# KrainskiL/CGE.jl

Measured on AMD Instinct MI355X. Metric: edge_alpha_evals_per_sec, higher is better.
Workload: dtype f64

## Files before the change

### cge.jl_amd/api.py

```python
from __future__ import annotations

import atexit
import ctypes as C
import os
import sys
import weakref

import numpy as np

from .args import _SplitRule

_HERE = os.path.dirname(os.path.abspath(__file__))
_LIB_PATH = os.path.join(_HERE, "csrc", "build", "libcge_hip.so")
_lib = None

CGE_OK = 0
_CODES = {-1: "AssertionError", -2: "ErrorException: Trying to split homogenous cluster",
          -3: "ErrorException: Unexpected empty cluster generated", -4: "HIP error / no GPU",
          -5: "collective hook failed", -6: "out of memory", -7: "bad argument"}


class CGEError(RuntimeError):
    def __init__(self, code, msg=""):
        super().__init__(f"{_CODES.get(code, 'error')} (code {code}){': ' + msg if msg else ''}")
# ... 423 lines not shown
        return out

    def segment_sort_test(self, z, offsets):
        z = _f64(z)
        off = np.ascontiguousarray(offsets, dtype=np.int32)
        zs, perm = np.empty_like(z), np.empty(z.size, dtype=np.int32)
        self._check(self.L.cge_segment_sort_test(self.h, _p(z), _p(off), C.c_int64(off.size - 1), _p(zs), _p(perm)))
        return zs, perm

    def wave_tree_test(self, x):
        x = np.ascontiguousarray(x, dtype=np.float64).reshape(-1, 64)
        a, b = np.empty(x.shape[0]), np.empty(x.shape[0])
        self._check(self.L.cge_wave_tree_test(self.h, _p(x), C.c_int64(x.shape[0]), _p(a), _p(b)))
        return a, b

    def js(self, vC, vB, vI=None, internal=True):
        vC, vB = _f64(vC), _f64(vB)
        vi = None if vI is None or len(vI) == 0 else np.ascontiguousarray(vI, dtype=np.uint8)
        out = C.c_double()
        self._check(self.L.cge_js(self.h, _p(vC), _p(vB), C.c_int64(len(vC)), _p(vi), C.c_int(int(bool(internal))),
                                  C.byref(out)))
        return out.value

    def exchange_buffer(self, min_doubles):
        ptr, cap = C.c_void_p(), C.c_int64()
        self._check(self.L.cge_exchange_buffer(self.h, C.c_int64(min_doubles), C.byref(ptr), C.byref(cap)))
        return ptr.value, cap.value

    def set_collectives(self, fn, rank, world):
        cb = ALLREDUCE_FN(fn)
# ... 173 lines not shown
```

### cge.jl_amd/csrc/capi.cpp

```cpp
#include <algorithm>
#include <cmath>
#include <future>
#include <thread>
#include <unordered_set>

#include "common.hpp"
#include "../../include/cge_hip_testing.h"
#include <limits>

void k_gather_i32(cge_ctx *c, const i32 *arr, const i32 *idx, i64 S, i32 *out);

#define CGE_TRY(ctx) try {
#define CGE_CATCH(ctx)                                             \
    }                                                              \
    catch (const CgeError &e) {                                    \
        if (ctx) (ctx)->err = e.msg;                               \
        return e.code;                                             \
    }                                                              \
    catch (const std::bad_alloc &) {                               \
        if (ctx) (ctx)->err = "host allocation failed";            \
        return CGE_E_OOM;                                          \
    }                                                              \
    catch (const std::exception &e) {                              \
        if (ctx) (ctx)->err = e.what();                            \
// ... 67 lines not shown
    try {
        HIP_CHECK(hipSetDevice(device));
        c->device = device;
        if (stream) {
            c->stream = (hipStream_t)stream;
        } else {
            HIP_CHECK(hipStreamCreateWithFlags(&c->stream, hipStreamNonBlocking));
            c->own_stream = true;
        }
        HIP_CHECK(hipStreamCreateWithFlags(&c->copy_stream, hipStreamNonBlocking));
        HIP_CHECK(hipEventCreateWithFlags(&c->copy_ev, hipEventDisableTiming));
        HIP_CHECK(hipEventCreateWithFlags(&c->copy_done, hipEventDisableTiming));
        for (int i = 0; i < 2; i++) HIP_CHECK(hipEventCreateWithFlags(&c->sweep_ev[i], hipEventDisableTiming));
        for (int i = 0; i < 2; i++) HIP_CHECK(hipEventCreateWithFlags(&c->tab_ev[i], hipEventDisableTiming));
        for (int i = 0; i < 2; i++) HIP_CHECK(hipEventCreateWithFlags(&c->stage_ev[i], hipEventDisableTiming));
        unsigned hc = std::thread::hardware_concurrency();
        c->n_threads = (int)std::max(1u, std::min(hc ? hc : 8u, 16u));
        c->pool = new ThreadPool(c->n_threads - 1);
        for (int b = 0; b < 2; b++) c->stage[b].ensure(CGE_STAGE_BYTES);
        {
            DevBuf<unsigned char> warm;
            warm.ensure((size_t)1 << 20);
            for (int b = 0; b < 2; b++) {
                memset(c->stage[b].p, 0, (size_t)1 << 20);
                HIP_CHECK(hipMemcpyAsync(warm.p, c->stage[b].p, (size_t)1 << 20, hipMemcpyHostToDevice, c->stream));
            }
            HIP_CHECK(hipStreamSynchronize(c->stream));
        }
        if (const char *nap = getenv("CGE_FIT_TEST_DELAY")) {
            c->opt_fit_test_delay = std::max(0, std::min(atoi(nap), 2000));
// ... 17 lines not shown
    flush_timers(c);
    (void)cge_comm_finalize(c);
    if (c->own_stream && c->stream) (void)hipStreamDestroy(c->stream);
    if (c->copy_stream) { (void)hipStreamSynchronize(c->copy_stream); (void)hipStreamDestroy(c->copy_stream); }
    for (hipEvent_t e : c->event_pool) (void)hipEventDestroy(e);
    c->event_pool.clear();
    if (c->copy_ev) (void)hipEventDestroy(c->copy_ev);
    if (c->copy_done) (void)hipEventDestroy(c->copy_done);
    if (c->samp_ev) (void)hipEventDestroy(c->samp_ev);
    for (int i = 0; i < 2; i++) {
        if (c->sweep_ev[i]) (void)hipEventDestroy(c->sweep_ev[i]);
        if (c->tab_ev[i]) (void)hipEventDestroy(c->tab_ev[i]);
    }
    for (int i = 0; i < 2; i++)
        if (c->stage_ev[i]) (void)hipEventDestroy(c->stage_ev[i]);
    delete c->pool;
    c->pool = nullptr;
    delete c;
}

const char *cge_last_error(const cge_ctx *c) { return c ? c->err.c_str() : "null context"; }

int cge_set_host_threads(cge_ctx *c, int n) {
    if (!c || n < 1) return CGE_E_ARG;
    c->n_threads = n;
    delete c->pool;
    c->pool = new ThreadPool(n - 1);
    return CGE_OK;
}

// ... 546 lines not shown
    if (method < 0 || method > 3) CGE_THROW(CGE_E_ARG, "unknown split method %d", method);
    const i64 d = c->d;
    hipStream_t st = c->stream;
    double t0 = now_ms();
    land = clamp_to_unique_rows(c, land, &c->lm_truncated);
    c->phases.ms["lm_unique"] = now_ms() - t0;
    if (c->after_unique) {
        std::function<void()> f;
        f.swap(c->after_unique);
        f();
    }
    std::vector<i64> gid;
    host_runsplit(c, cl_flat, cl_off, ncl, land, forced, method, gid, true);
    HIP_CHECK(hipStreamSynchronize(st));
    c->phases.ms["landmarks"] = now_ms() - t0;
    t0 = now_ms();
    const i64 N = (i64)c->h_mem_off.size() - 1;
    c->N = N;
    c->h_v2l.clear();
    c->lemb.ensure((size_t)N * d);
    c->lweight.ensure(N);
    c->dii.ensure(N);
    c->lcomm.ensure(N);
    {
        ScopedKernelTimer tm(c, "landmark_aggregate");
        k_landmark_aggregate(c, c->Xr.p, lm_vw(c), lm_comm(c), c->lm_memoff.p, c->lm_mem.p, N, d, c->lemb.p, c->lweight.p, c->dii.p,
                             c->lcomm.p);
    }
    if (c->rows_sharded) {
        DevBuf<double> &X = c->samp_xchg;
        const i64 words = N * (d + 3);
        X.ensure(words);
        k_pack_landmarks(c, c->lemb.p, c->lweight.p, c->dii.p, c->lcomm.p, N, d, X.p, 0);
        allreduce(c, X.p, words, 2);
        k_pack_landmarks(c, c->lemb.p, c->lweight.p, c->dii.p, c->lcomm.p, N, d, X.p, 1);
    }
    HIP_CHECK(hipStreamSynchronize(st));
    c->phases.ms["aggregate"] = now_ms() - t0;
    t0 = now_ms();
    const i64 C = c->n_comm_max;
    const i64 vlen = directed ? C * C : packed_len(C);
    c->vectC.ensure(vlen);
    scatter_vectC_resident(c, C, directed, c->vectC.p);
    c->lm_directed = directed;
    c->wedges_ready = false;
    c->n_ledges = -1;
    if (need_wedges) scatter_wedges(c, directed);
    HIP_CHECK(hipStreamSynchronize(st));
    c->phases.ms["scatter"] = now_ms() - t0;
    c->lm_ready = true;
}

int cge_landmarks_run(cge_ctx *c, const int64_t *cl_flat, const int64_t *cl_off, int64_t ncl, int64_t land,
                      int64_t forced, int method, int directed, int64_t *N_out, int64_t *n_ledges_out, int *truncated) {
    if (!c || !cl_flat || !cl_off) return CGE_E_ARG;
    CGE_TRY(c)
    HIP_CHECK(hipSetDevice(c->device));
    landmarks_run_impl(c, cl_flat, cl_off, ncl, land, forced, method, directed, true);
    if (N_out) *N_out = c->N;
    if (n_ledges_out) *n_ledges_out = c->n_ledges;
    if (truncated) *truncated = c->lm_truncated;
    CGE_CATCH(c)
}

// ... 368 lines not shown
            if (c->wedges_block_only) {
                const i64 per = wedge_rows_per_rank(c, N), r0 = std::min<i64>(N, per * c->coll.rank), r1 = std::min<i64>(N, r0 + per);
                DevBuf<double> &X = c->samp_xchg;
                X.ensure(3 * N);
                k_wedge_degrees_block(c, c->wedges.p, N, r0, r1, X.p);
                allreduce(c, X.p, 3 * N, 0);
                k_degrees_unpack(c, X.p, N, c->s_degout.p, c->s_degin.p, star.p);
            } else
                k_wedge_degrees(c, c->wedges.p, N, c->s_degout.p, c->s_degin.p, star.p);
            if (star_return(c, star.p, N, out, out_len)) return;
            G.deg_in = c->s_degin.p;
            G.deg_out = c->s_degout.p;
        }
        t0 = now_ms();
        ov = resident_orig_view(c, c->lweight.p);
        lcomm_host.resize(N);
        HIP_CHECK(hipMemcpyAsync(lcomm_host.data(), c->lcomm.p, sizeof(i32) * N, hipMemcpyDeviceToHost, st));
        HIP_CHECK(hipStreamSynchronize(st));
        ov.hi = host_diameter_landmarks(c, c->lemb.p, c->lweight.p, lcomm_host, C, N);
        ov.h_lcomm = lcomm_host.data();
        c->phases.ms["diameter"] = now_ms() - t0;
    } else {
        if (c->edges_sharded)
            CGE_THROW(CGE_E_ARG, "score: exact mode reads the whole edge list on every rank; the resident one is sharded (option shard_ingest)");
        if (c->rows_sharded)
            CGE_THROW(CGE_E_ARG, "score: exact mode reads every embedding row on every rank; the resident rows are sharded (option shard_rows)");
        const i64 N = c->n, C = c->n_comm_max;
        zeros.ensure(N);
        HIP_CHECK(hipMemsetAsync(zeros.p, 0, sizeof(double) * N, st));
        const i64 vlen = directed ? C * C : packed_len(C);
        c->vectC.ensure(vlen);
        scatter_vectC_resident(c, C, directed, c->vectC.p);
        G.N = N; G.d = d; G.C = C;
// ... 463 lines not shown
int cge_wave_tree_test(void *ctx, const double *x, int64_t n_rows, double *out_ref, double *out_new) {
    cge_ctx *c = (cge_ctx *)ctx;
    if (!c || !x || !out_ref || !out_new || n_rows <= 0) return CGE_E_ARG;
    CGE_TRY(c)
    HIP_CHECK(hipSetDevice(c->device));
    DevBuf<double> dx, da, db;
    dx.ensure((size_t)n_rows * 64); da.ensure(n_rows); db.ensure(n_rows);
    HIP_CHECK(hipMemcpyAsync(dx.p, x, sizeof(double) * n_rows * 64, hipMemcpyHostToDevice, c->stream));
    k_wave_tree_test(c, dx.p, n_rows, da.p, db.p);
    HIP_CHECK(hipMemcpyAsync(out_ref, da.p, sizeof(double) * n_rows, hipMemcpyDeviceToHost, c->stream));
    HIP_CHECK(hipMemcpyAsync(out_new, db.p, sizeof(double) * n_rows, hipMemcpyDeviceToHost, c->stream));
    HIP_CHECK(hipStreamSynchronize(c->stream));
    CGE_CATCH(c)
}

}

bool cge_exchange_fits(cge_ctx *c, size_t need) {
    if (c->xptr && need <= c->xcap) return true;
    if (!c->rccl_comm || (c->xptr && c->xptr != c->xown.p)) return false;
    c->xown.alloc_exact(std::max<size_t>(need + need / 4, 1 << 20));
    c->xptr = c->xown.p;
    c->xcap = c->xown.n;
    return true;
}

void cge_allgather_dev(cge_ctx *c, double *buf, i64 wpr) {
    if (!c->has_coll || wpr <= 0) return;
    if (c->rccl_comm && cge_rccl_allgather(c, buf, wpr)) return;
    const i64 W = c->coll.world, r = c->coll.rank, total = wpr * W;
// ... 20 lines not shown
```

### cge.jl_amd/csrc/common.hpp

```cpp
#pragma once
#include <hip/hip_runtime.h>

#include <algorithm>
#include <atomic>
#include <chrono>
#include <condition_variable>
#include <functional>
#include <mutex>
#include <thread>
#include <cstdint>
#include <cstdio>
#include <cstdlib>
#include <cstring>
#include <map>
#include <memory>
#include <string>
#include <vector>

#include "../../include/cge_hip.h"

typedef int64_t i64;
typedef int32_t i32;

struct MaxRec {
// ... 373 lines not shown
    DevBuf<i32> ls_rows, ls_row_task, ls_ct, ls_cb, ls_ce, ls_tco;
    DevBuf<double> ls_part, ls_mean, ls_sw, ls_cov, ls_vec, ls_z, ls_sums;
    DevBuf<unsigned char> ls_side, ls_state;
    DevBuf<double> ls_params;
    PinBuf<double> pin_sums, pin_params;
    PinBuf<i32> pin_clusters;
    PinBuf<i32> pin_hb_rows, pin_hb_row_task;
    DevBuf<i32> sp_srows, sp_meta, sp_rounds, sp_tro, sp_perm, sp_status, sort_idx, sort_idx2, sort_keys32, sort_k32b, sort_cnt;
    DevBuf<unsigned char> sort_keys8;
    DevBuf<i32> lm_arena;
    i64 lm_arena_used = 0;
    DevBuf<double> lm_means;
    i64 lm_means_used = 0;
    DevBuf<i64> ls_moff;
    PinBuf<i32> pin_tab[2], pin_res;
    DevBuf<i32> dev_tab, dev_res;
    hipEvent_t tab_ev[2] = {nullptr, nullptr};
    int tab_slot = 0;
    bool lm_index_on_device = false;
    DevBuf<i32> ls_toff, ls_nlow, lm_goff, lm_glen, lm_mem, lm_memoff;
    DevBuf<unsigned char> ls_keys;
    PinBuf<i32> pin_small;
    DevBuf<unsigned char> sort_tmp;
    DevBuf<unsigned long long> sort_k64;

    DevBuf<double> sp_zs, sp_ctot, sp_coff, sp_prefix, sp_vals;
    DevBuf<double> r2_F, r2_ck;
    i64 r2_rows = 0;

    int opt_landmark_edges = 0;
    DevBuf<i32> epd_i, s_star;
    DevBuf<i64> wed_cnt;
    DevBuf<double> cc_dense;
// ... 119 lines not shown
                  i64 n_tasks, i64 d, i32 *meta, i32 *rounds, double *vals, double *cmeans );
#define CGE_RR_MAXROUNDS 63
#define CGE_CHUNK_ROWS 1024
#define CGE_PARTIAL_BLOCKS 64
constexpr i64 RES_AUC = 0, RES_VERD = 2 * CGE_PARTIAL_BLOCKS, RES_JS = RES_VERD + 2, RES_FIT = RES_JS + 2 * CGE_PARTIAL_BLOCKS,
              RES_LEN = RES_FIT + 2, RES_STRIDE = RES_FIT + 16;
#define CGE_PREFIX_STRIDE 8
void k_gather_means(cge_ctx *c, const double *arena, const i64 *off, i64 T, i64 d, double *mean);
void k_gather_rows(cge_ctx *c, const i32 *arena, const i32 *task_off, const i32 *task_row_off, const i32 *chunk_task,
                   const i32 *chunk_beg, const i32 *chunk_end, i64 n_chunks, i32 *rows, i32 *row_task);
void k_rss_child_keys(cge_ctx *c, const i32 *perm, const i32 *row_task, const i32 *task_row_off, const i32 *meta,
                      const i32 *rounds, i64 R, i64 T, unsigned char *keys, i32 *nlow);
void k_side_counts(cge_ctx *c, const unsigned char *side, const i32 *task_row_off, i64 T, i32 *nlow);
void k_sort_children(cge_ctx *c, const unsigned char *keys, const i32 *rows, const i32 *task_row_off, const i32 *chunk_beg,
                     const i32 *chunk_end, const i32 *task_chunk_off, i64 n_chunks, i64 R, i64 T, int key_bits, i32 *out);
i64 k_groups_to_index(cge_ctx *c, const i32 *arena, const i32 *goff, const i32 *glen, i64 N, i64 n, i32 *v2l, i32 *mem);
void k_segmented_sort_z(cge_ctx *c, const double *z, const i32 *rows, const i32 *row_task, const i32 *task_row_off,
                        i64 R, i64 T, double *zs, i32 *perm, i32 *srows, i32 *status, i64 max_len = 0 );
void k_rss_side(cge_ctx *c, const double *z, const i32 *row_task, i64 n_rows, const double *params,
                unsigned char *state, unsigned char *side);
bool k_group_eig(cge_ctx *c, const double *cov, i64 n_tasks, i64 d, double *vec);
void k_group_project(cge_ctx *c, const double *Xr, const double *vw, const i32 *rows, const i32 *row_task, i64 n_rows,
                     i64 d, const double *mean, const double *vec, double *z);
void k_landmark_aggregate(cge_ctx *c, const double *Xr, const double *vw, const i32 *comm, const i32 *mem_off,
                          const i32 *mem, i64 N, i64 d, double *lemb, double *lweight, double *dii, i32 *lcomm);
bool k_edge_scatter_blocked_applies(const cge_ctx *c, i64 C);
bool k_blocked_edges_possible(const cge_ctx *c);
void k_pack_upper(cge_ctx *c, const double *dense, i64 C, double *packed);
bool k_build_blocked_edges(cge_ctx *c);
void k_edge_scatter_blocked(cge_ctx *c, i64 c0, i64 c1, i64 C, int directed, double *vectC);
bool k_wedge_scatter_blocked(cge_ctx *c, const i32 *v2l, i64 N, i64 c0, i64 c1, int directed, double *wedges, i64 *positive,
// ... 74 lines not shown
    void add(T *device, const T *host, i64 count) {
        static_assert(sizeof(T) % 4 == 0, "4-byte words");
        if (count <= 0) return;
        dst.push_back(device);
        src.push_back(host);
        words.push_back(count * (i64)(sizeof(T) / 4));
    }
    void flush() {
        if (dst.empty()) return;
        i64 tot = 0;
        for (i64 w : words) tot += w + (w & 1);
        const int slot = c->tab_slot;
        c->tab_slot ^= 1;
        HIP_CHECK(hipEventSynchronize(c->tab_ev[slot]));
        c->pin_tab[slot].ensure((size_t)tot);
        c->dev_tab.ensure((size_t)tot);
        i32 *h = c->pin_tab[slot].p;
        std::vector<const void *> dsrc(dst.size());
        i64 pos = 0;
        for (size_t q = 0; q < dst.size(); q++) {
            std::memcpy(h + pos, src[q], (size_t)words[q] * 4);
            dsrc[q] = c->dev_tab.p + pos;
            pos += words[q] + (words[q] & 1);
        }
        HIP_CHECK(hipMemcpyAsync(c->dev_tab.p, h, sizeof(i32) * (size_t)tot, hipMemcpyHostToDevice, c->stream));
        HIP_CHECK(hipEventRecord(c->tab_ev[slot], c->stream));
        for (size_t q0 = 0; q0 < dst.size(); q0 += CGE_WORD_SEGS) {
            const int n = (int)std::min<size_t>(CGE_WORD_SEGS, dst.size() - q0);
            k_copy_words(c, n, &dst[q0], &dsrc[q0], &words[q0]);
        }
        dst.clear(); src.clear(); words.clear();
    }
};
void k_gather_means_slots(cge_ctx *c, const double *arena, const i64 *off, const i64 *slot, i64 T, i64 d, i64 stride, i64 lead,
                          double *dst);
void k_pow_prepare(cge_ctx *c, const double *D, i64 N, bool upper_only, bool blocked = false);
void k_pow_matrix(cge_ctx *c, const double *D, i64 N, double alpha, double *GD, bool upper_only = false);
void k_pow_test(cge_ctx *c, const double *x, i64 n, double alpha, int method, double *out);
#define CGE_FLOW_NP 32
struct cge_fit_fused {
    const double *Lh; const float *Ll; double alpha;
    const i32 *comm, *fc, *ns, *base; double *partial;
    i64 S; const double *dpos, *dneg, *wts; const i32 *aidx; const double *afac, *aden; double *apw; double *auc_part;
};
bool k_fit_flow_enqueue(cge_ctx *c, const double *GD, i64 N, const double *T0, double *Tout, i64 Tld, const double *w,
                        double eps, double delta, int *dev_flags, const cge_fit_fused *ff = nullptr,
                        const cge_fit_fused *ff_dev = nullptr);
// ... 140 lines not shown
```

### cge.jl_amd/csrc/kernels_sort.hip

```cpp
#include <cstring>

#include "common.hpp"

#include <rocprim/rocprim.hpp>

using RadixOnly = rocprim::radix_sort_config<rocprim::default_config, rocprim::default_config, rocprim::default_config, 4096>;
static int sort_radix_mask() { return 1; }
template <class K, class V>
static hipError_t radix_pairs(void *tmp, size_t &bytes, const K *ki, K *ko, const V *vi, V *vo, size_t n, int b0, int b1,
                              hipStream_t st) {
    if (sort_radix_mask() & (sizeof(K) > 4 ? 2 : 1))
        return rocprim::radix_sort_pairs<RadixOnly>(tmp, bytes, ki, ko, vi, vo, n, b0, b1, st);
    return rocprim::radix_sort_pairs(tmp, bytes, ki, ko, vi, vo, n, b0, b1, st);
}
__global__ void iota_local_kernel(const i32 *__restrict__ row_task, const i32 *__restrict__ task_row_off, i64 R,
                                  i32 *__restrict__ idx) {
    const i64 j = (i64)blockIdx.x * blockDim.x + threadIdx.x;
    if (j < R) idx[j] = (i32)(j - task_row_off[row_task[j]]);
}
__global__ void sorted_gather_kernel(const i32 *__restrict__ rows, const i32 *__restrict__ row_task,
                                     const i32 *__restrict__ task_row_off, const i32 *__restrict__ perm, i64 R,
                                     i32 *__restrict__ srows) {
    const i64 j = (i64)blockIdx.x * blockDim.x + threadIdx.x;
    if (j < R) srows[j] = rows[task_row_off[row_task[j]] + perm[j]];
// ... 346 lines not shown

__global__ __launch_bounds__(256) void assign_groups_kernel(const i32 *__restrict__ arena, const i32 *__restrict__ goff,
                                                            const i32 *__restrict__ glen, i32 *__restrict__ v2l) {
    const i64 g = blockIdx.x;
    const i64 o = goff[g], k = glen[g];
    for (i64 q = threadIdx.x; q < k; q += 256) v2l[arena[o + q]] = (i32)g;
}
__global__ void count_unassigned_kernel(const i32 *__restrict__ v2l, i64 n, i32 *__restrict__ cnt) {
    const i64 i = (i64)blockIdx.x * blockDim.x + threadIdx.x;
    if (i < n && v2l[i] < 0) atomicAdd(cnt, 1);
}
__global__ void iota_kernel(i32 *__restrict__ x, i64 n) {
    const i64 i = (i64)blockIdx.x * blockDim.x + threadIdx.x;
    if (i < n) x[i] = (i32)i;
}
i64 k_groups_to_index(cge_ctx *c, const i32 *arena, const i32 *goff, const i32 *glen, i64 N, i64 n, i32 *v2l, i32 *mem) {
    hipStream_t st = c->stream;
    HIP_CHECK(hipMemsetAsync(v2l, 0xFF, sizeof(i32) * n, st));
    hipLaunchKernelGGL(assign_groups_kernel, dim3((unsigned)N), dim3(256), 0, st, arena, goff, glen, v2l);
    c->sort_cnt.ensure(1);
    HIP_CHECK(hipMemsetAsync(c->sort_cnt.p, 0, sizeof(i32), st));
    const unsigned nb = (unsigned)((n + 255) / 256);
    hipLaunchKernelGGL(count_unassigned_kernel, dim3(nb), dim3(256), 0, st, v2l, n, c->sort_cnt.p);
    c->sort_idx.ensure(n);
    c->sort_keys32.ensure(n);
    hipLaunchKernelGGL(iota_kernel, dim3(nb), dim3(256), 0, st, c->sort_idx.p, n);
    int bits = 1;
    while (((i64)1 << bits) < N) bits++;
    size_t bytes = 0;
    HIP_CHECK(radix_pairs(nullptr, bytes, (const unsigned *)v2l, (unsigned *)c->sort_keys32.p, c->sort_idx.p, mem,
                                        (size_t)n, 0, bits, st));
    c->sort_tmp.ensure(bytes);
    HIP_CHECK(radix_pairs(c->sort_tmp.p, bytes, (const unsigned *)v2l, (unsigned *)c->sort_keys32.p,
                                        c->sort_idx.p, mem, (size_t)n, 0, bits, st));
    i32 bad = 0;
    HIP_CHECK(hipMemcpyAsync(&bad, c->sort_cnt.p, sizeof(i32), hipMemcpyDeviceToHost, st));
    HIP_CHECK(hipStreamSynchronize(st));
    return bad;
}

__global__ void scatter_i32_kernel(const i32 *__restrict__ src, const i32 *__restrict__ idx, i64 cnt, i32 add, i32 *__restrict__ dst) {
    const i64 i = (i64)blockIdx.x * blockDim.x + threadIdx.x;
    if (i < cnt) dst[idx[i]] = src[i] + add;
}
__global__ void add_i32_kernel(const i32 *__restrict__ src, i64 n, i32 add, i32 *__restrict__ dst) {
    const i64 i = (i64)blockIdx.x * blockDim.x + threadIdx.x;
    if (i < n) dst[i] = src[i] + add;
}
void k_scatter_i32(cge_ctx *c, const i32 *src, const i32 *idx, i64 cnt, i32 add, i32 *dst) {
    if (cnt > 0) hipLaunchKernelGGL(scatter_i32_kernel, dim3((unsigned)((cnt + 255) / 256)), dim3(256), 0, c->stream, src, idx, cnt, add, dst);
}
void k_add_i32(cge_ctx *c, const i32 *src, i64 n, i32 add, i32 *dst) {
    if (n > 0) hipLaunchKernelGGL(add_i32_kernel, dim3((unsigned)((n + 255) / 256)), dim3(256), 0, c->stream, src, n, add, dst);
// ... 31 lines not shown
```

### cge.jl_amd/csrc/landmarks_host.cpp

```cpp
#include <algorithm>
#include <atomic>
#include <cfloat>
#include <cmath>
#include <memory>

#include "common.hpp"

namespace {

struct PhaseAcc {
    cge_ctx *c;
    const char *name;
    double t0;
    PhaseAcc(cge_ctx *ctx, const char *n) : c(ctx), name(n), t0(now_ms()) {}
    ~PhaseAcc() { c->phases.ms[name] += now_ms() - t0; }
};

struct Group {
    i64 off = -1, len = 0;
    std::vector<i64> what;
    double value = 0.0;
    bool has_split = false;
    int rc = CGE_OK;
    i64 coff = -1, nlow = 0;
// ... 296 lines not shown
        B.task_chunk_off[t] = (i32)B.chunk_task.size();
        const i64 k = lens[t];
        B.max_len = std::max(B.max_len, k);
        for (i64 s = 0; s < k; s += CH) {
            B.chunk_task.push_back((i32)t);
            B.chunk_beg.push_back((i32)(pos + s));
            B.chunk_end.push_back((i32)(pos + std::min(k, s + CH)));
        }
        pos += k;
    }
    B.R = pos;
    B.task_row_off[T] = (i32)pos;
    B.task_chunk_off[T] = (i32)B.chunk_task.size();
    B.NC = (i64)B.chunk_task.size();
}
struct WordGatherer {
    cge_ctx *c;
    std::vector<void *> ddst;
    std::vector<const void *> dsrc;
    std::vector<i64> words, offs;
    i64 tot = 0;
    explicit WordGatherer(cge_ctx *c_) : c(c_) {}
    template <class T>
    size_t add(const T *device, i64 count) {
        static_assert(sizeof(T) % 4 == 0, "4-byte words");
        dsrc.push_back(device);
        const i64 w = count * (i64)(sizeof(T) / 4);
        words.push_back(w);
        offs.push_back(tot);
        tot += w + (w & 1);
        return words.size() - 1;
    }
    void fetch() {
        fetch_async();
        wait();
    }
    void wait() { HIP_CHECK(hipEventSynchronize(c->copy_done)); }
    void fetch_async() {
        c->pin_res.ensure((size_t)std::max<i64>(tot, 1));
        c->dev_res.ensure((size_t)std::max<i64>(tot, 1));
        ddst.resize(dsrc.size());
        for (size_t q = 0; q < dsrc.size(); q++) ddst[q] = c->dev_res.p + offs[q];
        for (size_t q0 = 0; q0 < dsrc.size(); q0 += CGE_WORD_SEGS) {
            const int n = (int)std::min<size_t>(CGE_WORD_SEGS, dsrc.size() - q0);
            k_copy_words(c, n, &ddst[q0], &dsrc[q0], &words[q0]);
        }
        if (tot > 0)
            HIP_CHECK(hipMemcpyAsync(c->pin_res.p, c->dev_res.p, sizeof(i32) * (size_t)tot, hipMemcpyDeviceToHost, c->stream));
        HIP_CHECK(hipEventRecord(c->copy_done, c->stream));
    }
    template <class T>
    const T *get(size_t item) const { return reinterpret_cast<const T *>(c->pin_res.p + offs[item]); }
};
void upload_tables(cge_ctx *c, const Batch &B, WordPacker &pk) {
    const i64 d = c->d;
    c->ls_rows.ensure(B.R); c->ls_row_task.ensure(B.R); c->ls_ct.ensure(B.NC); c->ls_cb.ensure(B.NC);
    c->ls_ce.ensure(B.NC); c->ls_tco.ensure(B.T + 1); c->sp_tro.ensure(B.T + 1);
    c->ls_part.ensure((size_t)B.NC * std::max(d * d, 2 * (2 * d + 1)));
    c->ls_side.ensure(B.R);
    c->ls_sums.ensure((size_t)B.T * 2 * (2 * d + 1));
    pk.add(c->ls_ct.p, B.chunk_task.data(), B.NC);
    pk.add(c->ls_cb.p, B.chunk_beg.data(), B.NC);
    pk.add(c->ls_ce.p, B.chunk_end.data(), B.NC);
    pk.add(c->ls_tco.p, B.task_chunk_off.data(), B.T + 1);
    pk.add(c->sp_tro.p, B.task_row_off.data(), B.T + 1);
}
void build_batch(cge_ctx *c, Group *const *groups, i64 T, Batch &B) {
    std::vector<i64> lens(T);
// ... 272 lines not shown
    const double *vals = S.wg->get<double>(S.i_vals);
    for (i64 t = 0; t < T; t++) {
        Group *g = S.groups[t];
        S.nlow[t] = meta[2 * t] + 1;
        S.vlow[t] = vals[2 * t];
        S.vhigh[t] = vals[2 * t + 1];
        g->cmean_off = S.mbase + 2 * t * d;
        g->rc = CGE_OK;
        S.done[t] = 1;
    }
}

void rule_cut_enqueue(cge_ctx *c, SplitBatch &S, bool use_median) {
    const Batch &B = S.B;
    const i64 T = B.T, R = B.R, d = c->d;
    hipStream_t st = c->stream;
    if (use_median) {
        c->sp_srows.ensure(R); c->sp_zs.ensure(R); c->sp_perm.ensure(R); c->sp_status.ensure(T);
        k_segmented_sort_z(c, c->ls_z.p, c->ls_rows.p, c->ls_row_task.p, c->sp_tro.p, R, T, c->sp_zs.p, c->sp_perm.p,
                           c->sp_srows.p, c->sp_status.p, B.max_len);
    }
    c->ls_nlow.ensure(T);
    k_cut_sides(c, c->ls_z.p, use_median ? c->sp_zs.p : nullptr, c->sp_tro.p, T, use_median ? 1 : 0, c->ls_side.p, c->ls_nlow.p,
                c->cut_ties.p);
    c->pin_res.ensure((size_t)T);
    HIP_CHECK(hipMemcpyAsync(c->pin_res.p, c->ls_nlow.p, sizeof(i32) * T, hipMemcpyDeviceToHost, st));
    k_group_side_sums(c, c->Xr.p, lm_vw(c), c->ls_rows.p, c->ls_side.p, c->ls_cb.p, c->ls_ce.p, B.NC, c->ls_tco.p, B.T, d,
                      c->ls_part.p, c->ls_sums.p);
    c->sp_vals.ensure(2 * T);
    k_side_values_means(c, c->ls_sums.p, T, d, c->sp_vals.p, c->lm_means.p + S.mbase);
    c->pin_sums.ensure((size_t)2 * T);
    HIP_CHECK(hipMemcpyAsync(c->pin_sums.p, c->sp_vals.p, sizeof(double) * 2 * T, hipMemcpyDeviceToHost, st));
    HIP_CHECK(hipEventRecord(c->copy_done, st));
    k_sort_children(c, c->ls_side.p, c->ls_rows.p, c->sp_tro.p, c->ls_cb.p, c->ls_ce.p, c->ls_tco.p, B.NC, R, T, 2, c->lm_arena.p + S.base);
}
void rule_cut_collect(cge_ctx *c, SplitBatch &S) {
    const i64 T = S.B.T, d = c->d;
    HIP_CHECK(hipEventSynchronize(c->copy_done));
    const double *vals = c->pin_sums.p;
    std::memcpy(S.nlow.data(), c->pin_res.p, sizeof(i32) * T);
    for (i64 t = 0; t < T; t++) {
        Group *g = S.groups[t];
        S.vlow[t] = vals[2 * t];
        S.vhigh[t] = vals[2 * t + 1];
        g->cmean_off = S.mbase + 2 * t * d;
        g->rc = CGE_OK;
        S.done[t] = 1;
    }
}

void rss_generic_tasks(cge_ctx *c, SplitBatch &out, const std::vector<i64> &todo) {
    const Batch &B = out.B;
    Group *const *groups = out.groups;
    const i64 d = c->d, width = 2 * (2 * d + 1), base = out.base;
    hipStream_t st = c->stream;
// ... 703 lines not shown
            g->off = sc.a_off[cidx] >= 0 ? sc.a_off[cidx] + (t - cl_off[cidx]) : -1;
            g->len = 1;
            g->value = DBL_EPSILON;
            g->owner = sc.owner[cidx];
            H.put(g);
        }
    }
}

void final_index(cge_ctx *c, const Heap &H, std::vector<i64> &group_ids, bool want_index) {
    PhaseAcc pfin(c, "lm_final");
    const i64 n = c->n, NG = (i64)H.len(), nrows = lm_rows(c);
    const bool RS = c->rows_sharded;
    const int me = RS ? c->coll.rank : 0;
    hipStream_t st = c->stream;
    c->pin_small.ensure((size_t)2 * NG + 2);
    i32 *goff = c->pin_small.p, *glen = goff + NG;
    c->h_mem_off.assign(NG + 1, 0);
    c->h_gl_off.assign(NG + 1, 0);
    c->lm_owner.assign(NG, 0);
    for (i64 g = 0; g < NG; g++) {
        const Group *G = H.at(g + 1);
        const bool mine = !RS || G->owner == me;
        goff[g] = mine ? (i32)G->off : 0;
        glen[g] = mine ? (i32)G->len : 0;
        c->h_mem_off[g + 1] = c->h_mem_off[g] + glen[g];
        c->h_gl_off[g + 1] = c->h_gl_off[g] + (i32)G->len;
        c->lm_owner[g] = G->owner;
    }
    DevBuf<i32> &v2l_rows = RS ? c->v2l_loc : c->v2l;
    c->lm_goff.ensure(NG); c->lm_glen.ensure(NG); c->v2l.ensure(n); v2l_rows.ensure(nrows); c->lm_mem.ensure(nrows); c->lm_memoff.ensure(NG + 1);
    HIP_CHECK(hipMemcpyAsync(c->lm_goff.p, goff, sizeof(i32) * NG, hipMemcpyHostToDevice, st));
    HIP_CHECK(hipMemcpyAsync(c->lm_glen.p, glen, sizeof(i32) * NG, hipMemcpyHostToDevice, st));
    HIP_CHECK(hipMemcpyAsync(c->lm_memoff.p, c->h_mem_off.data(), sizeof(i32) * (NG + 1), hipMemcpyHostToDevice, st));
    const i64 unassigned = k_groups_to_index(c, c->lm_arena.p, c->lm_goff.p, c->lm_glen.p, NG, nrows, v2l_rows.p, c->lm_mem.p);
    bool cover_bad = unassigned != 0 || c->h_mem_off[NG] != nrows || c->h_gl_off[NG] != n;
    if (RS) {
        const i64 words = (n + 1) / 2;
        DevBuf<i32> &tmp = c->sort_idx2;
        tmp.ensure(2 * words);
        HIP_CHECK(hipMemsetAsync(tmp.p, 0, sizeof(i32) * 2 * words, st));
        k_scatter_i32(c, v2l_rows.p, c->loc2glob.p, nrows, 1, tmp.p);
        cge_allreduce_dev(c, reinterpret_cast<double *>(tmp.p), words, 2);
        k_add_i32(c, tmp.p, n, -1, c->v2l.p);
        std::vector<double> verdict(1, cover_bad ? 1.0 : 0.0);
        exchange_group_words(c, verdict);
        cover_bad = verdict[0] != 0.0;
    }
    if (cover_bad)
        CGE_THROW(CGE_E_ASSERT, "AssertionError: all(>=(0), group_ids) [%lld rows without a group, %lld of %lld rows in the groups here, %lld of %lld over all ranks]",
                  (long long)unassigned, (long long)c->h_mem_off[NG], (long long)nrows, (long long)c->h_gl_off[NG], (long long)n);
    c->lm_index_on_device = want_index;
    c->h_mem.clear();
    if (want_index) {
        HIP_CHECK(hipStreamSynchronize(st));
        group_ids.clear();
        return;
    }
    c->h_v2l0.resize(n);
    HIP_CHECK(hipMemcpyAsync(c->h_v2l0.data(), c->v2l.p, sizeof(i32) * n, hipMemcpyDeviceToHost, st));
    HIP_CHECK(hipStreamSynchronize(st));
    group_ids.resize(n);
    parallel_for(c, 64, [&](i64 part) {
        for (i64 i = n * part / 64; i < n * (part + 1) / 64; i++) group_ids[i] = c->h_v2l0[i];
    });
}

}

void host_runsplit(cge_ctx *c, const i64 *cl_flat, const i64 *cl_off, i64 ncl, i64 nland, i64 forced, int method,
                   std::vector<i64> &group_ids, bool want_index) {
    if (!c->Xr.p || c->Xr.n < (size_t)(lm_rows(c) * c->d) || (i64)c->h_vw.size() != c->n)
        CGE_THROW(CGE_E_ARG, "runsplit: embedding / vertex weights are not resident");
    GroupPool pool;
    Heap H;
    std::vector<i64> order;
// ... 25 lines not shown
```

### include/cge_hip_testing.h

```cpp
#ifndef CGE_HIP_TESTING_H
#define CGE_HIP_TESTING_H
#include <stdint.h>
#ifdef __cplusplus
extern "C" {
#endif
int cge_host_eig_top(const double *A, int64_t d, double *v);
int cge_batch_pack_test(const int64_t *N, int64_t K, int cus, int32_t *group_of);
int cge_host_pos_draw(int64_t seed, int64_t stream_id, int64_t S, int64_t m, int64_t *pos_idx);
int cge_group_eig(void *ctx, const double *A, int64_t T, int64_t d, double *v);
int cge_diameter_bounds_test(void *ctx, const int64_t *v2l, int64_t N, const int64_t *lcomm, int64_t C, int pass, double *P,
                             int64_t *nref, int *pass_ran, double *ref_points, double *mean);
int cge_pow_test(void *ctx, const double *x, int64_t n, double alpha, int method, double *out);
int cge_rccl_selftest(void *ctx, double *host_inout, int64_t count, int op);
int cge_segment_sort_test(void *ctx, const double *z, const int32_t *task_row_off, int64_t T, double *zs_out, int32_t *perm_out);
int cge_wave_tree_test(void *ctx, const double *x, int64_t n_rows, double *out_ref, double *out_new);
int cge_set_test_option(void *ctx, const char *key, int64_t value);
#ifdef __cplusplus
}
#endif
#endif
```

Baseline: 11.71 billion.

## Let copy kernels read and write pinned host memory directly, dropping staging hops

Result: no change. 11.67 billion (-0.3%).

```diff
diff --git a/cge.jl_amd/api.py b/cge.jl_amd/api.py
--- a/cge.jl_amd/api.py
+++ b/cge.jl_amd/api.py
@@ -461,6 +461,15 @@
         self._check(self.L.cge_wave_tree_test(self.h, _p(x), C.c_int64(x.shape[0]), _p(a), _p(b)))
         return a, b
 
+    def word_roundtrip_test(self, items):
+        items = [np.ascontiguousarray(a, dtype=np.int32).ravel() for a in items]
+        off = np.zeros(len(items) + 1, dtype=np.int64)
+        off[1:] = np.cumsum([len(a) for a in items])
+        flat = np.ascontiguousarray(np.concatenate(items + [np.zeros(1, np.int32)]))
+        out = np.full(len(flat), -7, dtype=np.int32)
+        self._check(self.L.cge_word_roundtrip_test(self.h, _p(flat), _p(off), C.c_int64(len(items)), _p(out)))
+        return [out[off[q]:off[q + 1]].copy() for q in range(len(items))]
+
     def js(self, vC, vB, vI=None, internal=True):
         vC, vB = _f64(vC), _f64(vB)
         vi = None if vI is None or len(vI) == 0 else np.ascontiguousarray(vI, dtype=np.uint8)
diff --git a/cge.jl_amd/csrc/capi.cpp b/cge.jl_amd/csrc/capi.cpp
--- a/cge.jl_amd/csrc/capi.cpp
+++ b/cge.jl_amd/csrc/capi.cpp
@@ -105,6 +105,7 @@
         for (int i = 0; i < 2; i++) HIP_CHECK(hipEventCreateWithFlags(&c->sweep_ev[i], hipEventDisableTiming));
         for (int i = 0; i < 2; i++) HIP_CHECK(hipEventCreateWithFlags(&c->tab_ev[i], hipEventDisableTiming));
         for (int i = 0; i < 2; i++) HIP_CHECK(hipEventCreateWithFlags(&c->stage_ev[i], hipEventDisableTiming));
+        for (int i = 0; i < 3; i++) HIP_CHECK(hipEventCreate(&c->phase_ev[i]));
         unsigned hc = std::thread::hardware_concurrency();
         c->n_threads = (int)std::max(1u, std::min(hc ? hc : 8u, 16u));
         c->pool = new ThreadPool(c->n_threads - 1);
@@ -152,6 +153,8 @@
     }
     for (int i = 0; i < 2; i++)
         if (c->stage_ev[i]) (void)hipEventDestroy(c->stage_ev[i]);
+    for (int i = 0; i < 3; i++)
+        if (c->phase_ev[i]) (void)hipEventDestroy(c->phase_ev[i]);
     delete c->pool;
     c->pool = nullptr;
     delete c;
@@ -728,7 +731,7 @@
     host_runsplit(c, cl_flat, cl_off, ncl, land, forced, method, gid, true);
     HIP_CHECK(hipStreamSynchronize(st));
     c->phases.ms["landmarks"] = now_ms() - t0;
-    t0 = now_ms();
+    HIP_CHECK(hipEventRecord(c->phase_ev[0], st));
     const i64 N = (i64)c->h_mem_off.size() - 1;
     c->N = N;
     c->h_v2l.clear();
@@ -749,9 +752,9 @@
         allreduce(c, X.p, words, 2);
         k_pack_landmarks(c, c->lemb.p, c->lweight.p, c->dii.p, c->lcomm.p, N, d, X.p, 1);
     }
-    HIP_CHECK(hipStreamSynchronize(st));
-    c->phases.ms["aggregate"] = now_ms() - t0;
-    t0 = now_ms();
+    c->pin_lcomm.ensure(N);
+    HIP_CHECK(hipMemcpyAsync(c->pin_lcomm.p, c->lcomm.p, sizeof(i32) * N, hipMemcpyDeviceToHost, st));
+    HIP_CHECK(hipEventRecord(c->phase_ev[1], st));
     const i64 C = c->n_comm_max;
     const i64 vlen = directed ? C * C : packed_len(C);
     c->vectC.ensure(vlen);
@@ -760,8 +763,13 @@
     c->wedges_ready = false;
     c->n_ledges = -1;
     if (need_wedges) scatter_wedges(c, directed);
+    HIP_CHECK(hipEventRecord(c->phase_ev[2], st));
     HIP_CHECK(hipStreamSynchronize(st));
-    c->phases.ms["scatter"] = now_ms() - t0;
+    float ms_agg = 0.f, ms_sc = 0.f;
+    HIP_CHECK(hipEventElapsedTime(&ms_agg, c->phase_ev[0], c->phase_ev[1]));
+    HIP_CHECK(hipEventElapsedTime(&ms_sc, c->phase_ev[1], c->phase_ev[2]));
+    c->phases.ms["aggregate"] = ms_agg;
+    c->phases.ms["scatter"] = ms_sc;
     c->lm_ready = true;
 }
 
@@ -1160,9 +1168,7 @@
         }
         t0 = now_ms();
         ov = resident_orig_view(c, c->lweight.p);
-        lcomm_host.resize(N);
-        HIP_CHECK(hipMemcpyAsync(lcomm_host.data(), c->lcomm.p, sizeof(i32) * N, hipMemcpyDeviceToHost, st));
-        HIP_CHECK(hipStreamSynchronize(st));
+        lcomm_host.assign(c->pin_lcomm.p, c->pin_lcomm.p + N);
         ov.hi = host_diameter_landmarks(c, c->lemb.p, c->lweight.p, lcomm_host, C, N);
         ov.h_lcomm = lcomm_host.data();
         c->phases.ms["diameter"] = now_ms() - t0;
@@ -1656,6 +1662,28 @@
     CGE_CATCH(c)
 }
 
+int cge_word_roundtrip_test(void *ctx, const int32_t *words, const int64_t *item_off, int64_t n_items, int32_t *out) {
+    cge_ctx *c = (cge_ctx *)ctx;
+    if (!c || !words || !item_off || !out || n_items <= 0) return CGE_E_ARG;
+    CGE_TRY(c)
+    HIP_CHECK(hipSetDevice(c->device));
+    const i64 total = item_off[n_items];
+    DevBuf<i32> dev;
+    dev.ensure((size_t)total);
+    HIP_CHECK(hipMemsetAsync(dev.p, 0xFF, sizeof(i32) * (size_t)std::max<i64>(total, 1), c->stream));
+    WordPacker pk(c);
+    WordGatherer wg(c);
+    for (i64 q = 0; q < n_items; q++) {
+        pk.add(dev.p + item_off[q], words + item_off[q], item_off[q + 1] - item_off[q]);
+        wg.add(dev.p + item_off[q], item_off[q + 1] - item_off[q]);
+    }
+    pk.flush();
+    wg.fetch();
+    for (i64 q = 0; q < n_items; q++)
+        std::memcpy(out + item_off[q], wg.get<i32>((size_t)q), sizeof(i32) * (size_t)(item_off[q + 1] - item_off[q]));
+    CGE_CATCH(c)
+}
+
 }
 
 bool cge_exchange_fits(cge_ctx *c, size_t need) {
diff --git a/cge.jl_amd/csrc/common.hpp b/cge.jl_amd/csrc/common.hpp
--- a/cge.jl_amd/csrc/common.hpp
+++ b/cge.jl_amd/csrc/common.hpp
@@ -411,9 +411,10 @@
     i64 lm_means_used = 0;
     DevBuf<i64> ls_moff;
     PinBuf<i32> pin_tab[2], pin_res;
-    DevBuf<i32> dev_tab, dev_res;
     hipEvent_t tab_ev[2] = {nullptr, nullptr};
     int tab_slot = 0;
+    hipEvent_t phase_ev[3] = {nullptr, nullptr, nullptr};
+    PinBuf<i32> pin_lcomm;
     bool lm_index_on_device = false;
     DevBuf<i32> ls_toff, ls_nlow, lm_goff, lm_glen, lm_mem, lm_memoff;
     DevBuf<unsigned char> ls_keys;
@@ -563,7 +564,7 @@
 void k_side_counts(cge_ctx *c, const unsigned char *side, const i32 *task_row_off, i64 T, i32 *nlow);
 void k_sort_children(cge_ctx *c, const unsigned char *keys, const i32 *rows, const i32 *task_row_off, const i32 *chunk_beg,
                      const i32 *chunk_end, const i32 *task_chunk_off, i64 n_chunks, i64 R, i64 T, int key_bits, i32 *out);
-i64 k_groups_to_index(cge_ctx *c, const i32 *arena, const i32 *goff, const i32 *glen, i64 N, i64 n, i32 *v2l, i32 *mem);
+void k_groups_to_index(cge_ctx *c, const i32 *arena, const i32 *goff, const i32 *glen, i64 N, i64 n, i32 *v2l, i32 *mem, i32 *unassigned);
 void k_segmented_sort_z(cge_ctx *c, const double *z, const i32 *rows, const i32 *row_task, const i32 *task_row_off,
                         i64 R, i64 T, double *zs, i32 *perm, i32 *srows, i32 *status, i64 max_len = 0 );
 void k_rss_side(cge_ctx *c, const double *z, const i32 *row_task, i64 n_rows, const double *params,
@@ -668,23 +669,56 @@
         c->tab_slot ^= 1;
         HIP_CHECK(hipEventSynchronize(c->tab_ev[slot]));
         c->pin_tab[slot].ensure((size_t)tot);
-        c->dev_tab.ensure((size_t)tot);
         i32 *h = c->pin_tab[slot].p;
-        std::vector<const void *> dsrc(dst.size());
+        std::vector<const void *> psrc(dst.size());
         i64 pos = 0;
         for (size_t q = 0; q < dst.size(); q++) {
             std::memcpy(h + pos, src[q], (size_t)words[q] * 4);
-            dsrc[q] = c->dev_tab.p + pos;
+            psrc[q] = h + pos;
             pos += words[q] + (words[q] & 1);
         }
-        HIP_CHECK(hipMemcpyAsync(c->dev_tab.p, h, sizeof(i32) * (size_t)tot, hipMemcpyHostToDevice, c->stream));
-        HIP_CHECK(hipEventRecord(c->tab_ev[slot], c->stream));
         for (size_t q0 = 0; q0 < dst.size(); q0 += CGE_WORD_SEGS) {
             const int n = (int)std::min<size_t>(CGE_WORD_SEGS, dst.size() - q0);
-            k_copy_words(c, n, &dst[q0], &dsrc[q0], &words[q0]);
-        }
+            k_copy_words(c, n, &dst[q0], &psrc[q0], &words[q0]);
+        }
+        HIP_CHECK(hipEventRecord(c->tab_ev[slot], c->stream));
         dst.clear(); src.clear(); words.clear();
     }
+};
+struct WordGatherer {
+    cge_ctx *c;
+    std::vector<void *> pdst;
+    std::vector<const void *> dsrc;
+    std::vector<i64> words, offs;
+    i64 tot = 0;
+    explicit WordGatherer(cge_ctx *c_) : c(c_) {}
+    template <class T>
+    size_t add(const T *device, i64 count) {
+        static_assert(sizeof(T) % 4 == 0, "4-byte words");
+        dsrc.push_back(device);
+        const i64 w = count * (i64)(sizeof(T) / 4);
+        words.push_back(w);
+        offs.push_back(tot);
+        tot += w + (w & 1);
+        return words.size() - 1;
+    }
+    void fetch() {
+        fetch_async();
+        wait();
+    }
+    void wait() { HIP_CHECK(hipEventSynchronize(c->copy_done)); }
+    void fetch_async() {
+        c->pin_res.ensure((size_t)std::max<i64>(tot, 1));
+        pdst.resize(dsrc.size());
+        for (size_t q = 0; q < dsrc.size(); q++) pdst[q] = c->pin_res.p + offs[q];
+        for (size_t q0 = 0; q0 < dsrc.size(); q0 += CGE_WORD_SEGS) {
+            const int n = (int)std::min<size_t>(CGE_WORD_SEGS, dsrc.size() - q0);
+            k_copy_words(c, n, &pdst[q0], &dsrc[q0], &words[q0]);
+        }
+        HIP_CHECK(hipEventRecord(c->copy_done, c->stream));
+    }
+    template <class T>
+    const T *get(size_t item) const { return reinterpret_cast<const T *>(c->pin_res.p + offs[item]); }
 };
 void k_gather_means_slots(cge_ctx *c, const double *arena, const i64 *off, const i64 *slot, i64 T, i64 d, i64 stride, i64 lead,
                           double *dst);
diff --git a/cge.jl_amd/csrc/kernels_sort.hip b/cge.jl_amd/csrc/kernels_sort.hip
--- a/cge.jl_amd/csrc/kernels_sort.hip
+++ b/cge.jl_amd/csrc/kernels_sort.hip
@@ -384,7 +384,7 @@
     const i64 i = (i64)blockIdx.x * blockDim.x + threadIdx.x;
     if (i < n) x[i] = (i32)i;
 }
-i64 k_groups_to_index(cge_ctx *c, const i32 *arena, const i32 *goff, const i32 *glen, i64 N, i64 n, i32 *v2l, i32 *mem) {
+void k_groups_to_index(cge_ctx *c, const i32 *arena, const i32 *goff, const i32 *glen, i64 N, i64 n, i32 *v2l, i32 *mem, i32 *unassigned) {
     hipStream_t st = c->stream;
     HIP_CHECK(hipMemsetAsync(v2l, 0xFF, sizeof(i32) * n, st));
     hipLaunchKernelGGL(assign_groups_kernel, dim3((unsigned)N), dim3(256), 0, st, arena, goff, glen, v2l);
@@ -403,10 +403,7 @@
     c->sort_tmp.ensure(bytes);
     HIP_CHECK(radix_pairs(c->sort_tmp.p, bytes, (const unsigned *)v2l, (unsigned *)c->sort_keys32.p,
                                         c->sort_idx.p, mem, (size_t)n, 0, bits, st));
-    i32 bad = 0;
-    HIP_CHECK(hipMemcpyAsync(&bad, c->sort_cnt.p, sizeof(i32), hipMemcpyDeviceToHost, st));
-    HIP_CHECK(hipStreamSynchronize(st));
-    return bad;
+    HIP_CHECK(hipMemcpyAsync(unassigned, c->sort_cnt.p, sizeof(i32), hipMemcpyDeviceToHost, st));
 }
 
 __global__ void scatter_i32_kernel(const i32 *__restrict__ src, const i32 *__restrict__ idx, i64 cnt, i32 add, i32 *__restrict__ dst) {
diff --git a/cge.jl_amd/csrc/landmarks_host.cpp b/cge.jl_amd/csrc/landmarks_host.cpp
--- a/cge.jl_amd/csrc/landmarks_host.cpp
+++ b/cge.jl_amd/csrc/landmarks_host.cpp
@@ -334,44 +334,6 @@
     B.task_chunk_off[T] = (i32)B.chunk_task.size();
     B.NC = (i64)B.chunk_task.size();
 }
-struct WordGatherer {
-    cge_ctx *c;
-    std::vector<void *> ddst;
-    std::vector<const void *> dsrc;
-    std::vector<i64> words, offs;
-    i64 tot = 0;
-    explicit WordGatherer(cge_ctx *c_) : c(c_) {}
-    template <class T>
-    size_t add(const T *device, i64 count) {
-        static_assert(sizeof(T) % 4 == 0, "4-byte words");
-        dsrc.push_back(device);
-        const i64 w = count * (i64)(sizeof(T) / 4);
-        words.push_back(w);
-        offs.push_back(tot);
-        tot += w + (w & 1);
-        return words.size() - 1;
-    }
-    void fetch() {
-        fetch_async();
-        wait();
-    }
-    void wait() { HIP_CHECK(hipEventSynchronize(c->copy_done)); }
-    void fetch_async() {
-        c->pin_res.ensure((size_t)std::max<i64>(tot, 1));
-        c->dev_res.ensure((size_t)std::max<i64>(tot, 1));
-        ddst.resize(dsrc.size());
-        for (size_t q = 0; q < dsrc.size(); q++) ddst[q] = c->dev_res.p + offs[q];
-        for (size_t q0 = 0; q0 < dsrc.size(); q0 += CGE_WORD_SEGS) {
-            const int n = (int)std::min<size_t>(CGE_WORD_SEGS, dsrc.size() - q0);
-            k_copy_words(c, n, &ddst[q0], &dsrc[q0], &words[q0]);
-        }
-        if (tot > 0)
-            HIP_CHECK(hipMemcpyAsync(c->pin_res.p, c->dev_res.p, sizeof(i32) * (size_t)tot, hipMemcpyDeviceToHost, c->stream));
-        HIP_CHECK(hipEventRecord(c->copy_done, c->stream));
-    }
-    template <class T>
-    const T *get(size_t item) const { return reinterpret_cast<const T *>(c->pin_res.p + offs[item]); }
-};
 void upload_tables(cge_ctx *c, const Batch &B, WordPacker &pk) {
     const i64 d = c->d;
     c->ls_rows.ensure(B.R); c->ls_row_task.ensure(B.R); c->ls_ct.ensure(B.NC); c->ls_cb.ensure(B.NC);
@@ -674,7 +636,6 @@
 void rule_cut_enqueue(cge_ctx *c, SplitBatch &S, bool use_median) {
     const Batch &B = S.B;
     const i64 T = B.T, R = B.R, d = c->d;
-    hipStream_t st = c->stream;
     if (use_median) {
         c->sp_srows.ensure(R); c->sp_zs.ensure(R); c->sp_perm.ensure(R); c->sp_status.ensure(T);
         k_segmented_sort_z(c, c->ls_z.p, c->ls_rows.p, c->ls_row_task.p, c->sp_tro.p, R, T, c->sp_zs.p, c->sp_perm.p,
@@ -683,22 +644,20 @@
     c->ls_nlow.ensure(T);
     k_cut_sides(c, c->ls_z.p, use_median ? c->sp_zs.p : nullptr, c->sp_tro.p, T, use_median ? 1 : 0, c->ls_side.p, c->ls_nlow.p,
                 c->cut_ties.p);
-    c->pin_res.ensure((size_t)T);
-    HIP_CHECK(hipMemcpyAsync(c->pin_res.p, c->ls_nlow.p, sizeof(i32) * T, hipMemcpyDeviceToHost, st));
     k_group_side_sums(c, c->Xr.p, lm_vw(c), c->ls_rows.p, c->ls_side.p, c->ls_cb.p, c->ls_ce.p, B.NC, c->ls_tco.p, B.T, d,
                       c->ls_part.p, c->ls_sums.p);
     c->sp_vals.ensure(2 * T);
     k_side_values_means(c, c->ls_sums.p, T, d, c->sp_vals.p, c->lm_means.p + S.mbase);
-    c->pin_sums.ensure((size_t)2 * T);
-    HIP_CHECK(hipMemcpyAsync(c->pin_sums.p, c->sp_vals.p, sizeof(double) * 2 * T, hipMemcpyDeviceToHost, st));
-    HIP_CHECK(hipEventRecord(c->copy_done, st));
+    S.wg.reset(new WordGatherer(c));
+    S.i_nlow = S.wg->add(c->ls_nlow.p, T); S.i_vals = S.wg->add(c->sp_vals.p, 2 * T);
+    S.wg->fetch_async();
     k_sort_children(c, c->ls_side.p, c->ls_rows.p, c->sp_tro.p, c->ls_cb.p, c->ls_ce.p, c->ls_tco.p, B.NC, R, T, 2, c->lm_arena.p + S.base);
 }
 void rule_cut_collect(cge_ctx *c, SplitBatch &S) {
     const i64 T = S.B.T, d = c->d;
-    HIP_CHECK(hipEventSynchronize(c->copy_done));
-    const double *vals = c->pin_sums.p;
-    std::memcpy(S.nlow.data(), c->pin_res.p, sizeof(i32) * T);
+    S.wg->wait();
+    const double *vals = S.wg->get<double>(S.i_vals);
+    std::memcpy(S.nlow.data(), S.wg->get<i32>(S.i_nlow), sizeof(i32) * T);
     for (i64 t = 0; t < T; t++) {
         Group *g = S.groups[t];
         S.vlow[t] = vals[2 * t];
@@ -1432,8 +1391,7 @@
     const bool RS = c->rows_sharded;
     const int me = RS ? c->coll.rank : 0;
     hipStream_t st = c->stream;
-    c->pin_small.ensure((size_t)2 * NG + 2);
-    i32 *goff = c->pin_small.p, *glen = goff + NG;
+    std::vector<i32> goff(NG), glen(NG);
     c->h_mem_off.assign(NG + 1, 0);
     c->h_gl_off.assign(NG + 1, 0);
     c->lm_owner.assign(NG, 0);
@@ -1448,11 +1406,22 @@
     }
     DevBuf<i32> &v2l_rows = RS ? c->v2l_loc : c->v2l;
     c->lm_goff.ensure(NG); c->lm_glen.ensure(NG); c->v2l.ensure(n); v2l_rows.ensure(nrows); c->lm_mem.ensure(nrows); c->lm_memoff.ensure(NG + 1);
-    HIP_CHECK(hipMemcpyAsync(c->lm_goff.p, goff, sizeof(i32) * NG, hipMemcpyHostToDevice, st));
-    HIP_CHECK(hipMemcpyAsync(c->lm_glen.p, glen, sizeof(i32) * NG, hipMemcpyHostToDevice, st));
-    HIP_CHECK(hipMemcpyAsync(c->lm_memoff.p, c->h_mem_off.data(), sizeof(i32) * (NG + 1), hipMemcpyHostToDevice, st));
-    const i64 unassigned = k_groups_to_index(c, c->lm_arena.p, c->lm_goff.p, c->lm_glen.p, NG, nrows, v2l_rows.p, c->lm_mem.p);
-    bool cover_bad = unassigned != 0 || c->h_mem_off[NG] != nrows || c->h_gl_off[NG] != n;
+    {
+        WordPacker pk(c);
+        pk.add(c->lm_goff.p, goff.data(), NG);
+        pk.add(c->lm_glen.p, glen.data(), NG);
+        pk.add(c->lm_memoff.p, c->h_mem_off.data(), NG + 1);
+        pk.flush();
+    }
+    c->pin_small.ensure(1);
+    k_groups_to_index(c, c->lm_arena.p, c->lm_goff.p, c->lm_glen.p, NG, nrows, v2l_rows.p, c->lm_mem.p, c->pin_small.p);
+    i64 unassigned = 0;
+    bool cover_bad = c->h_mem_off[NG] != nrows || c->h_gl_off[NG] != n;
+    auto settle = [&]() {
+        HIP_CHECK(hipStreamSynchronize(st));
+        unassigned = c->pin_small.p[0];
+        cover_bad = cover_bad || unassigned != 0;
+    };
     if (RS) {
         const i64 words = (n + 1) / 2;
         DevBuf<i32> &tmp = c->sort_idx2;
@@ -1461,9 +1430,16 @@
         k_scatter_i32(c, v2l_rows.p, c->loc2glob.p, nrows, 1, tmp.p);
         cge_allreduce_dev(c, reinterpret_cast<double *>(tmp.p), words, 2);
         k_add_i32(c, tmp.p, n, -1, c->v2l.p);
+        settle();
         std::vector<double> verdict(1, cover_bad ? 1.0 : 0.0);
         exchange_group_words(c, verdict);
         cover_bad = verdict[0] != 0.0;
+    } else {
+        if (!want_index) {
+            c->h_v2l0.resize(n);
+            HIP_CHECK(hipMemcpyAsync(c->h_v2l0.data(), c->v2l.p, sizeof(i32) * n, hipMemcpyDeviceToHost, st));
+        }
+        settle();
     }
     if (cover_bad)
         CGE_THROW(CGE_E_ASSERT, "AssertionError: all(>=(0), group_ids) [%lld rows without a group, %lld of %lld rows in the groups here, %lld of %lld over all ranks]",
@@ -1471,13 +1447,14 @@
     c->lm_index_on_device = want_index;
     c->h_mem.clear();
     if (want_index) {
-        HIP_CHECK(hipStreamSynchronize(st));
         group_ids.clear();
         return;
     }
-    c->h_v2l0.resize(n);
-    HIP_CHECK(hipMemcpyAsync(c->h_v2l0.data(), c->v2l.p, sizeof(i32) * n, hipMemcpyDeviceToHost, st));
-    HIP_CHECK(hipStreamSynchronize(st));
+    if (RS) {
+        c->h_v2l0.resize(n);
+        HIP_CHECK(hipMemcpyAsync(c->h_v2l0.data(), c->v2l.p, sizeof(i32) * n, hipMemcpyDeviceToHost, st));
+        HIP_CHECK(hipStreamSynchronize(st));
+    }
     group_ids.resize(n);
     parallel_for(c, 64, [&](i64 part) {
         for (i64 i = n * part / 64; i < n * (part + 1) / 64; i++) group_ids[i] = c->h_v2l0[i];
diff --git a/include/cge_hip_testing.h b/include/cge_hip_testing.h
--- a/include/cge_hip_testing.h
+++ b/include/cge_hip_testing.h
@@ -14,6 +14,7 @@
 int cge_rccl_selftest(void *ctx, double *host_inout, int64_t count, int op);
 int cge_segment_sort_test(void *ctx, const double *z, const int32_t *task_row_off, int64_t T, double *zs_out, int32_t *perm_out);
 int cge_wave_tree_test(void *ctx, const double *x, int64_t n_rows, double *out_ref, double *out_new);
+int cge_word_roundtrip_test(void *ctx, const int32_t *words, const int64_t *item_off, int64_t n_items, int32_t *out);
 int cge_set_test_option(void *ctx, const char *key, int64_t value);
 #ifdef __cplusplus
 }
diff --git a/profiles/microbench_hop.hip b/profiles/microbench_hop.hip
--- /dev/null
+++ b/profiles/microbench_hop.hip
@@ -0,0 +1,76 @@
+#include <hip/hip_runtime.h>
+#include <algorithm>
+#include <chrono>
+#include <cstdio>
+#include <cstdlib>
+#include <cstring>
+#include <vector>
+#define CK(x) do { hipError_t e_ = (x); if (e_ != hipSuccess) { printf("%s: %s\n", #x, hipGetErrorString(e_)); exit(1); } } while (0)
+static double now_us() { return std::chrono::duration<double, std::micro>(std::chrono::steady_clock::now().time_since_epoch()).count(); }
+__global__ void produce(unsigned *out, int n, unsigned seed) {
+    for (int i = threadIdx.x; i < n; i += blockDim.x) out[i] = seed + (unsigned)i;
+}
+__global__ void copy_words(unsigned *dst, const unsigned *src, int n) {
+    for (int i = blockIdx.x * blockDim.x + threadIdx.x; i < n; i += gridDim.x * blockDim.x) dst[i] = src[i];
+}
+__global__ void consume(const unsigned *in, int n, unsigned *sum) {
+    unsigned s = 0;
+    for (int i = threadIdx.x; i < n; i += blockDim.x) s += in[i];
+    atomicAdd(sum, s);
+}
+static void report(const char *what, std::vector<double> &t) {
+    std::sort(t.begin(), t.end());
+    printf("%-78s median %7.1f us   min %7.1f us\n", what, t[t.size() / 2], t[0]);
+}
+int main() {
+    const int T = 512, W = 6 * T, REP = 200;
+    hipStream_t st;
+    CK(hipStreamCreateWithFlags(&st, hipStreamNonBlocking));
+    hipEvent_t ev;
+    CK(hipEventCreateWithFlags(&ev, hipEventDisableTiming));
+    unsigned *d_src, *d_stage, *d_tab, *d_sum, *pin;
+    CK(hipMalloc(&d_src, W * 4)); CK(hipMalloc(&d_stage, W * 4)); CK(hipMalloc(&d_tab, W * 4)); CK(hipMalloc(&d_sum, 4));
+    CK(hipHostMalloc(&pin, W * 4, hipHostMallocDefault));
+    std::vector<unsigned> host(W);
+    std::vector<double> t(REP);
+    const int nb = (W + 255) / 256;
+    for (int path = 0; path < 2; path++) {
+        for (int r = -10; r < REP; r++) {
+            const double t0 = now_us();
+            hipLaunchKernelGGL(produce, dim3(1), dim3(256), 0, st, d_src, W, (unsigned)r);
+            if (path == 0) {
+                hipLaunchKernelGGL(copy_words, dim3(nb), dim3(256), 0, st, d_stage, d_src, W);
+                CK(hipMemcpyAsync(pin, d_stage, W * 4, hipMemcpyDeviceToHost, st));
+            } else
+                hipLaunchKernelGGL(copy_words, dim3(nb), dim3(256), 0, st, pin, d_src, W);
+            CK(hipEventRecord(ev, st));
+            CK(hipEventSynchronize(ev));
+            if (pin[W - 1] != (unsigned)r + (unsigned)(W - 1)) { printf("wrong result on the host\n"); return 1; }
+            if (r >= 0) t[r] = now_us() - t0;
+        }
+        report(path == 0 ? "(r1) results: gather -> device staging -> copy to pinned -> event" : "(r2) results: gather writes pinned memory -> event", t);
+    }
+    for (int path = 0; path < 2; path++) {
+        for (int r = -10; r < REP; r++) {
+            for (int i = 0; i < W; i++) host[i] = (unsigned)(r + i);
+            CK(hipMemsetAsync(d_sum, 0, 4, st));
+            CK(hipStreamSynchronize(st));
+            const double t0 = now_us();
+            memcpy(pin, host.data(), W * 4);
+            if (path == 0) {
+                CK(hipMemcpyAsync(d_stage, pin, W * 4, hipMemcpyHostToDevice, st));
+                hipLaunchKernelGGL(copy_words, dim3(nb), dim3(256), 0, st, d_tab, d_stage, W);
+            } else
+                hipLaunchKernelGGL(copy_words, dim3(nb), dim3(256), 0, st, d_tab, pin, W);
+            hipLaunchKernelGGL(consume, dim3(1), dim3(256), 0, st, d_tab, W, d_sum);
+            CK(hipStreamSynchronize(st));
+            if (r >= 0) t[r] = now_us() - t0;
+            unsigned got = 0, exp = 0;
+            CK(hipMemcpy(&got, d_sum, 4, hipMemcpyDeviceToHost));
+            for (int i = 0; i < W; i++) exp += host[i];
+            if (got != exp) { printf("wrong table on the device\n"); return 1; }
+        }
+        report(path == 0 ? "(t1) tables: pinned -> copy to device staging -> scatter -> consumer" : "(t2) tables: scatter reads pinned memory -> consumer", t);
+    }
+    return 0;
+}
```
